# Beryl2000/SE-UNet-AirSeg

Measured on AMD Instinct MI355X. Metric: voxels/sec SE-UNet fwd+bwd, 128^3 patch, higher is better.
Workload: dtype bf16

## Files before the change

### include/seunet_hip.h

```cpp
#ifndef SEUNET_HIP_H
#define SEUNET_HIP_H
#include <stddef.h>

#ifdef __cplusplus
extern "C" {
#endif

#ifndef SEUNET_F32
#define SEUNET_F32 0
#define SEUNET_BF16 1
#define SEUNET_F16 2
#endif
#define SEUNET_CONV_MFMA 0
#define SEUNET_CONV_NAIVE 1
#define SEUNET_CONV_MARCH 2
#define SEUNET_CONV_TILED 3

typedef void* seunet_stream_t;
typedef struct seunet_dims { int n, d, h, w; } seunet_dims;

int seunet_version(void);
const char* seunet_last_error(void);
int seunet_init(int device);

// ... 50 lines not shown
                             const float* pgrad_partial, int records, float* dw_se, float* dw_se2, float* dw_side,
                             float* db_side, float* dhead_w, seunet_stream_t s);

int seunet_cat_epilogue_fwd(int dtype, const void* raw, const float* mean, const float* rstd, const void* raw2,
                            const float* mean2, const float* rstd2, int c, float slope, void* out, seunet_dims dims,
                            seunet_stream_t s);
int seunet_cat_epilogue_bwd(int dtype, const void* g_out, const void* raw, const float* mean, const float* rstd,
                            const void* raw2, const float* mean2, const float* rstd2, int c, float slope,
                            const float* m1, const float* m2, const float* m1b, const float* m2b, void* dx, void* dx2,
                            double* stat_partial, double* stat_partial2, seunet_dims dims, seunet_stream_t s);

int seunet_xbranch_moment_slots(seunet_dims dims);
int seunet_xbranch_moments(int dtype, const void* x_in, double* partial , seunet_dims dims, seunet_stream_t s);
int seunet_xbranch_stats(const double* partial, int slots, const float* w2, int c, int in_channel, int n, long long count,
                         float eps, float* mean2, float* rstd2, double* moments_out , seunet_stream_t s);
int seunet_cat_epilogue_fwd_x(int dtype, const void* raw, const float* mean, const float* rstd, const void* x_in,
                              const float* w2, int in_channel, const float* mean2, const float* rstd2, int c, float slope,
                              void* out, seunet_dims dims, seunet_stream_t s);
int seunet_cat_epilogue_bwd_x(int dtype, const void* g_out, const void* raw, const float* mean, const float* rstd,
                              const void* x_in, const float* w2, int in_channel, const float* mean2, const float* rstd2,
                              int c, float slope, const float* m1, const float* m2, const float* m1b, const float* m2b,
                              void* dx, double* stat_partial, double* stat_partial2, double* xw_partial, seunet_dims dims,
                              seunet_stream_t s);
int seunet_cat_epilogue_fwd_x_pool(int dtype, const void* raw, const float* mean, const float* rstd, const void* x_in,
                                   const float* w2, int in_channel, const float* mean2, const float* rstd2, int c, float slope,
                                   void* out, void* pooled, unsigned int* argmax, seunet_dims dims, seunet_stream_t s);
int seunet_cat_epilogue_bwd_x_pool(int dtype, const void* g_out, const void* raw, const float* mean, const float* rstd,
                                   const void* x_in, const float* w2, int in_channel, const float* mean2, const float* rstd2,
                                   int c, float slope, const float* m1, const float* m2, const float* m1b, const float* m2b,
                                   void* dx, double* stat_partial, double* stat_partial2, double* xw_partial,
// ... 235 lines not shown
```

### se-unet-airseg_amd/_lib.py

```python
from __future__ import annotations

import ctypes as C
import os
from typing import Optional, Sequence

_HERE = os.path.dirname(os.path.abspath(__file__))
LIB_PATH = os.environ.get("SEUNET_LIB") or os.path.join(_HERE, "libseunet_hip.so")

F32, BF16, F16 = 0, 1, 2
CONV_MFMA, CONV_NAIVE, CONV_MARCH, CONV_TILED = 0, 1, 2, 3
LOSS_NSUMS = 7
DTI_F64, DTI_F32 = 0, 1
CC_EVALUATION, CC_MAXIMUM_3D, CC_LARGEST_FILLED = 0, 1, 2
MORPH_DILATE, MORPH_ERODE_BORDER0, MORPH_ERODE_BORDER1, MORPH_CLOSE = 0, 1, 2, 3


class Dims(C.Structure):
    _fields_ = [("n", C.c_int), ("d", C.c_int), ("h", C.c_int), ("w", C.c_int)]


class NetDesc(C.Structure):
    _fields_ = [("batch", C.c_int), ("in_channel", C.c_int), ("n_classes", C.c_int),
                ("d", C.c_int), ("h", C.c_int), ("w", C.c_int), ("width_mult", C.c_int),
                ("dtype", C.c_int), ("conv_impl", C.c_int),
# ... 58 lines not shown
    "seunet_head_bwd_tmp_floats": (_sz, [Dims]),
    "seunet_head_bwd": (_i, [_vp, _pp, _i, _vp, _vp, Dims, _vp]),
    "seunet_loss_partial_floats": (_i, []),
    "seunet_loss_sums": (_i, [_vp, _i, _vp, _vp, _vp, _ll, _vp, _vp, _i, _vp]),
    "seunet_loss_value": (_i, [_vp, _d, _d, _d, _vp, _d, _d, _d, _vp, _vp]),
    "seunet_loss_grad": (_i, [_vp, _i, _vp, _vp, _vp, _ll, _vp, _f, _f, _f, _f, _vp, _vp, _vp]),
    "seunet_loss_sample_partial_floats": (_i, [_i]),
    "seunet_loss_sums_per_sample": (_i, [_vp, _i, _vp, _vp, _vp, _i, _ll, _vp, _vp, _i, _vp]),
    "seunet_loss_sample_values": (_i, [_vp, _i, _d, _d, _d, _vp, _vp]),
    "seunet_pool_select": (_i, [_vp, _i, _vp, _vp, _vp, _i, _vp, _vp]),
    "seunet_pool_scatter": (_i, [_vp, _i, _i, _ll, _vp, _vp, _vp, _vp, _vp, _vp, _vp, _vp, _vp]),
    "seunet_pool_gather": (_i, [_ip, _i, _i, _ll, _vp, _vp, _vp, _vp, _vp, _vp, _vp, _vp, _vp]),
    "seunet_xbranch_moment_slots": (_i, [Dims]),
    "seunet_xbranch_moments": (_i, [_i, _vp, _vp, Dims, _vp]),
    "seunet_xbranch_stats": (_i, [_vp, _i, _vp, _i, _i, _i, _ll, _f, _vp, _vp, _vp, _vp]),
    "seunet_cat_epilogue_fwd_x": (_i, [_i, _vp, _vp, _vp, _vp, _vp, _i, _vp, _vp, _i, _f, _vp, Dims, _vp]),
    "seunet_cat_epilogue_bwd_x": (_i, [_i, _vp, _vp, _vp, _vp, _vp, _vp, _i, _vp, _vp, _i, _f, _vp, _vp, _vp, _vp, _vp, _vp, _vp, _vp, Dims, _vp]),
    "seunet_cat_epilogue_fwd_x_pool": (_i, [_i, _vp, _vp, _vp, _vp, _vp, _i, _vp, _vp, _i, _f, _vp, _vp, _vp, Dims, _vp]),
    "seunet_cat_epilogue_bwd_x_pool": (_i, [_i, _vp, _vp, _vp, _vp, _vp, _vp, _i, _vp, _vp, _i, _f, _vp, _vp, _vp, _vp, _vp, _vp, _vp, _vp, _vp, _vp, Dims, _vp]),
    "seunet_cat_xgrad_finalize": (_i, [_vp, _vp, _i, _vp, _vp, _i, _i, _i, _f, _vp, _vp]),
    "seunet_cc_workspace_bytes": (_sz, [_i, _i, _i]),
    "seunet_largest_component": (_i, [_vp, _i, _i, _i, _i, _vp, _vp, _vp, _sz, _vp]),
    "seunet_metric_out_bytes": (_sz, [_i]),
    "seunet_metric_sums": (_i, [_vp, _vp, _vp, _vp, _ll, _i, _vp, _sz, _vp]),
    "seunet_value_counts": (_i, [_vp, _ll, _i, _vp, _vp]),
    "seunet_shift_clamp": (_i, [_vp, _ll, _i, _i, _i, _i, _vp, _vp]),
    "seunet_get_l_workspace_bytes": (_sz, [_i, _i, _i]),
    "seunet_get_l": (_i, [_vp, _i, _i, _i, _d, _i, _vp, _vp, _sz, _vp]),
    "seunet_mask_combine": (_i, [_vp, _vp, _ll, _i, _vp, _vp]),
    "seunet_mask_box": (_i, [_vp, _i, _i, _i, _vp, _vp]),
    "seunet_crop3d": (_i, [_vp, _i, _i, _i, _i, _ip, _vp, _vp]),
# ... 126 lines not shown
```

### se-unet-airseg_amd/csrc/abi.cpp

```cpp
#include "seunet_common.h"
#include "epilogue.h"
#include "volume.h"
#include "wgrad.h"
#include "../../include/seunet_hip.h"

using namespace seunet;

static inline Dims D(seunet_dims d) { return Dims{d.n, d.d, d.h, d.w}; }
static inline hipStream_t S(seunet_stream_t s) { return reinterpret_cast<hipStream_t>(s); }

static int make_src(int nsrc, const void* const* src, const int* src_c, SrcList& l) {
  SEUNET_CHECK(nsrc >= 1 && nsrc <= 3 && src && src_c, "bad source list");
  l = SrcList{};
  l.n = nsrc;
  for (int i = 0; i < nsrc; ++i) { l.ptr[i] = src[i]; l.C[i] = src_c[i]; }
  return 0;
}

namespace seunet { extern unsigned long long* g_conv_debug; }

extern "C" {

int seunet_debug_set_buffer(void* p) { seunet::g_conv_debug = reinterpret_cast<unsigned long long*>(p); return 0; }
int seunet_debug_upsample2_form(int dtype, int c, seunet_dims dims, int backward) { return upsample2_form(dtype, c, D(dims), backward != 0); }
// ... 297 lines not shown
                       float* label_out, float* weight_out, float* skel_out, seunet_stream_t s) {
  return launch_pool_gather(slots_host, n, capacity, voxels, pool_data, pool_label, pool_weight, pool_skel, data_out, label_out,
                            weight_out, skel_out, S(s));
}

int seunet_xbranch_moment_slots(seunet_dims dims) { return xbranch_moment_slots(D(dims)); }
int seunet_xbranch_moments(int dtype, const void* x_in, double* partial, seunet_dims dims, seunet_stream_t s) {
  SEUNET_CHECK(x_in && partial, "xbranch_moments: null argument");
  return launch_xbranch_moments(dtype, x_in, partial, D(dims), S(s));
}
int seunet_xbranch_stats(const double* partial, int slots, const float* w2, int c, int in_channel, int n, long long count,
                         float eps, float* mean2, float* rstd2, double* moments_out, seunet_stream_t s) {
  SEUNET_CHECK(partial && w2 && mean2 && rstd2 && slots >= 1 && c >= 1 && n >= 1 && count >= 1, "xbranch_stats: bad argument");
  return launch_xbranch_stats(partial, slots, w2, c, in_channel, n, count, eps, mean2, rstd2, moments_out, S(s));
}
int seunet_cat_epilogue_fwd_x(int dtype, const void* raw, const float* mean, const float* rstd, const void* x_in,
                              const float* w2, int in_channel, const float* mean2, const float* rstd2, int c, float slope,
                              void* out, seunet_dims dims, seunet_stream_t s) {
  SEUNET_CHECK(raw && mean && rstd && x_in && w2 && mean2 && rstd2 && out, "cat_epilogue_fwd_x: null argument");
  const CatBlock b{{raw, mean, rstd}, {Branch2::Recomputed, x_in, mean2, rstd2, w2, in_channel}, c, slope};
  return launch_cat_fwd(dtype, b, out, PoolOut{}, D(dims), S(s));
}
int seunet_cat_epilogue_bwd_x(int dtype, const void* g_out, const void* raw, const float* mean, const float* rstd,
                              const void* x_in, const float* w2, int in_channel, const float* mean2, const float* rstd2,
                              int c, float slope, const float* m1, const float* m2, const float* m1b, const float* m2b,
                              void* dx, double* stat_partial, double* stat_partial2, double* xw_partial, seunet_dims dims,
                              seunet_stream_t s) {
  SEUNET_CHECK(g_out && raw && mean && rstd && x_in && w2 && mean2 && rstd2, "cat_epilogue_bwd_x: null argument");
  const CatBlock b{{raw, mean, rstd}, {Branch2::Recomputed, x_in, mean2, rstd2, w2, in_channel}, c, slope};
  return cat_epilogue_bwd(dtype, b, g_out, PoolGrad{}, m1, m2, m1b, m2b, dx, nullptr, stat_partial, stat_partial2, xw_partial, dims, s);
// ... 288 lines not shown
```

### se-unet-airseg_amd/csrc/cat.hip

```cpp
#include "epilogue.h"
#include "wgrad.h"
#include <type_traits>

namespace seunet {

template <bool XR>
__device__ __forceinline__ void second_branch(const float (&in8)[8], const float (&wa)[8], const float (&wb)[8], float (&x2)[8]) {
#pragma unroll
  for (int j = 0; j < 8; ++j) x2[j] = XR ? wa[j] * in8[0] + wb[j] * in8[1] : in8[j];
}

template <typename T, int LPV, bool TWO, bool XR>
__global__ void __launch_bounds__(EPI_THREADS)
cat_fwd_kernel(const T* __restrict__ raw, const float* __restrict__ mean, const float* __restrict__ rstd,
               const T* __restrict__ raw2, const float* __restrict__ mean2, const float* __restrict__ rstd2, int C, float slope,
               T* __restrict__ out, long long V, const float* __restrict__ w2x, int xic) {
  SEUNET_EPI_THREAD(LPV);
  float mu[8], rs[8], mu2[8], rs2[8], wa[8], wb[8];
#pragma unroll
  for (int j = 0; j < 8; ++j) {
    mu[j] = mean[n * C + c0 + j]; rs[j] = rstd[n * C + c0 + j];
    mu2[j] = TWO ? mean2[n * C + c0 + j] : 0.f;
    rs2[j] = TWO ? rstd2[n * C + c0 + j] : 0.f;
    wa[j] = XR ? w2x[(c0 + j) * xic] : 0.f;
// ... 255 lines not shown
__global__ void __launch_bounds__(EPI_THREADS)
input_moments_kernel(const T* __restrict__ xin, double* __restrict__ partial, long long V) {
  const int n = blockIdx.y, P = gridDim.x;
  double s[5] = {0.0, 0.0, 0.0, 0.0, 0.0};
  for (long long v = (long long)blockIdx.x * EPI_THREADS + threadIdx.x; v < V; v += (long long)P * EPI_THREADS) {
    float x[8];
    load8(xin + ((long long)n * V + v) * 8, x);
    const double a = (double)x[0], b = (double)x[1];
    s[0] += a; s[1] += b; s[2] += a * a; s[3] += a * b; s[4] += b * b;
  }
  __shared__ double red[4][5];
  block_sum(s, red);
  if (const int k = threadIdx.x; k < 5) partial[((long long)n * P + blockIdx.x) * 5 + k] = wave4_sum(red, k);
}

__global__ void __launch_bounds__(256)
xbranch_stats_kernel(const double* __restrict__ partial, int slots, const float* __restrict__ w2, int C, int ic,
                     double inv_count, float eps, float* __restrict__ mean2, float* __restrict__ rstd2,
                     double* __restrict__ moments_out) {
  const int n = blockIdx.x;
  __shared__ double red[4][5], tot[5];
  double s[5] = {0.0, 0.0, 0.0, 0.0, 0.0};
  for (int b = threadIdx.x; b < slots; b += 256)
#pragma unroll
    for (int k = 0; k < 5; ++k) s[k] += partial[((long long)n * slots + b) * 5 + k];
  block_sum(s, red);
  if (threadIdx.x < 5) tot[threadIdx.x] = wave4_sum(red, threadIdx.x) * inv_count;
  __syncthreads();
  if (moments_out != nullptr && threadIdx.x < 5) moments_out[n * 5 + threadIdx.x] = tot[threadIdx.x];
  const double m0 = tot[0], m1 = tot[1];
  const double c00 = tot[2] - m0 * m0, c01 = tot[3] - m0 * m1, c11 = tot[4] - m1 * m1;
  for (int c = threadIdx.x; c < C; c += 256) {
    const double a = (double)w2[c * ic], b = ic > 1 ? (double)w2[c * ic + 1] : 0.0;
    const double mu = a * m0 + b * m1;
    double var = a * a * c00 + 2.0 * a * b * c01 + b * b * c11;
    if (var < 0.0) var = 0.0;
    mean2[n * C + c] = (float)mu;
    rstd2[n * C + c] = (float)(1.0 / sqrt(var + (double)eps));
  }
}

__device__ __forceinline__ void
xw_finalize_body(int c, const double* __restrict__ xw_partial, const double* __restrict__ stat_partial2, int slots, int C, int N,
                 const double* __restrict__ moments, const float* __restrict__ w2, int ic, double eps, float* __restrict__ dw) {
  const int wave = threadIdx.x >> 6, lane = threadIdx.x & 63;
  __shared__ double red[4][3];
  const double wa = (double)w2[c * ic], wb = ic > 1 ? (double)w2[c * ic + 1] : 0.0;
  double g0 = 0.0, g1 = 0.0;
  for (int n = 0; n < N; ++n) {
    double s[3] = {0.0, 0.0, 0.0};
    for (int r = threadIdx.x; r < slots; r += 256) {
      const long long rec = (long long)n * slots + r;
      s[0] += xw_partial[(rec * C + c) * 2 + 0];
      s[1] += xw_partial[(rec * C + c) * 2 + 1];
// ... 171 lines not shown
int launch_xbranch_moments(int dtype, const void* x_in, double* partial, Dims d, hipStream_t s) {
  dim3 grid(xbranch_moment_slots(d), d.N);
  SEUNET_DTYPE_SWITCH(dtype, input_moments_kernel<T><<<grid, EPI_THREADS, 0, s>>>((const T*)x_in, partial, d.vox()));
  SEUNET_LAUNCH_CHECK();
  return 0;
}

int launch_xbranch_stats(const double* partial, int slots, const float* w2, int C, int in_channel, int N, long long count,
                         float eps, float* mean2, float* rstd2, double* moments_out, hipStream_t s) {
  SEUNET_CHECK(in_channel >= 1 && in_channel <= 2, "xbranch_stats: in_channel %d (1 or 2)", in_channel);
  xbranch_stats_kernel<<<N, 256, 0, s>>>(partial, slots, w2, C, in_channel, 1.0 / (double)count, eps, mean2, rstd2, moments_out);
  SEUNET_LAUNCH_CHECK();
  return 0;
}

int launch_cat_xgrad_finalize(const double* xw_partial, const double* stat_partial2, int slots, const double* moments, const float* w2,
                              int C, int in_channel, int N, float eps, float* dw, hipStream_t s) {
  SEUNET_CHECK(in_channel >= 1 && in_channel <= 2, "cat_xgrad_finalize: in_channel %d (1 or 2)", in_channel);
  xw_finalize_kernel<<<C, 256, 0, s>>>(xw_partial, stat_partial2, slots, C, N, moments, w2, in_channel, (double)eps, dw);
  SEUNET_LAUNCH_CHECK();
  return 0;
}

int launch_cat_bwd_finalize(const double* stat_partial, const double* stat_partial2, int slots, int C, int N, long long count,
                            float* m1, float* m2, float* m1b, float* m2b, const CatXwFinalize& xw, hipStream_t s,
                            const WgReduceJob* rider) {
  SEUNET_CHECK(stat_partial && m1 && m2 && (!stat_partial2 || (m1b && m2b)), "cat_bwd_finalize: missing argument");
  SEUNET_CHECK(!xw.dw || (stat_partial2 && xw.xw_partial && xw.moments && xw.w2 && xw.in_channel >= 1 && xw.in_channel <= 2),
               "cat_bwd_finalize: the x-branch weight gradient needs the second branch's sums and in_channel 1 or 2");
  const WgReduceJob job = rider ? *rider : WgReduceJob{};
// ... 19 lines not shown
```

### se-unet-airseg_amd/csrc/epilogue.h

```cpp
#pragma once
#include "seunet_common.h"

namespace seunet {

struct WgReduceJob;
int epi_partials(Dims d);
int launch_channel_stats(int dtype, const void* t, int C, double* partial, Dims d, hipStream_t s);
int launch_stats_finalize(const double* partial, int slots, int C, int N, long long count,
                          float eps, int mode, float* out_a, float* out_b, hipStream_t s);
struct NormIn { const void* raw; const float* mean; const float* rstd; };
struct SseParams {
  const float* w_se;
  const float* w_se2;
  const float* w_side;
  const float* b_side;
  float slope;
};
struct GateBlock { NormIn a; int C; SseParams p; };
struct SseHead {
  float* side_out;
  float* level_map;
  int level_accumulate;
  const float* head_w;
  const float* drop;
// ... 37 lines not shown
  const float *m1, *m2, *m1b, *m2b;
  void* dx;
  void* dx2;
  float* gx_out;
  int gx_acc;
};
int launch_cat_fwd(int dtype, const CatBlock& b, void* out, const PoolOut& pool, Dims d, hipStream_t s);
int launch_cat_bwd_sums(int dtype, const CatBlock& b, const void* g_out, const PoolGrad& pool, const CatSums& out, Dims d,
                        hipStream_t s);
int launch_cat_bwd_apply(int dtype, const CatBlock& b, const void* g_out, const PoolGrad& pool, const CatApply& io, Dims d,
                         hipStream_t s);
int xbranch_moment_slots(Dims d);
int launch_xbranch_moments(int dtype, const void* x_in, double* partial, Dims d, hipStream_t s);
int launch_xbranch_stats(const double* partial, int slots, const float* w2, int C, int in_channel, int N, long long count,
                         float eps, float* mean2, float* rstd2, double* moments_out, hipStream_t s);
int launch_cat_xgrad_finalize(const double* xw_partial, const double* stat_partial2, int slots, const double* moments, const float* w2,
                              int C, int in_channel, int N, float eps, float* dw, hipStream_t s);
struct CatXwFinalize { const double* xw_partial; const double* moments; const float* w2; int in_channel; float eps; float* dw; };
int launch_cat_bwd_finalize(const double* stat_partial, const double* stat_partial2, int slots, int C, int N, long long count,
                            float* m1, float* m2, float* m1b, float* m2b, const CatXwFinalize& xw, hipStream_t s,
                            const WgReduceJob* rider = nullptr);
int launch_xbranch_values(int dtype, const void* x_in, const float* w2, int C, int in_channel, float* out_ncdhw, Dims d, hipStream_t s);

#ifdef __HIPCC__
static constexpr int EPI_THREADS = 256;

template <typename T> __device__ __forceinline__ float round_to(float v) {
  if constexpr (sizeof(T) == 4) return v;
  else return unpack_lo<T>(pack2<T>(v, 0.f));
}
// ... 87 lines not shown
```

### se-unet-airseg_amd/csrc/net.cpp

```cpp
#include "seunet_common.h"
#include "epilogue.h"
#include "wgrad.h"
#include "../../include/seunet_hip.h"

#include <algorithm>
#include <cstdio>
#include <cstring>
#include <string>
#include <vector>

namespace seunet {

ConvKernel wgrad_kernel(int dtype, int taps, int dil, const SrcList& x, int cin_logical, int cout, Dims d, long long src_dist) {
  if (taps == 1) {
    const int combos = cdiv(cin_logical, 32) * cdiv(cout, 32);
    const long long nv = (long long)d.N * d.vox();
    const bool pays = combos >= 16 || (combos >= 8 && nv >= 500000);
    return pays && wgrad_1x1_supported(dtype, x, cin_logical, cout) ? ConvKernel::Wgrad1x1 : ConvKernel::Tiled;
  }
  const bool fine = d.W >= 32 && (long long)d.D * d.H * d.W >= 48LL * 48 * 48;
  const bool pays = fine || dil == 2 || cin_logical >= 256;
  return pays && wgrad_march_supported(dtype, taps, dil, x, cin_logical, cout, d, src_dist) ? ConvKernel::March : ConvKernel::Tiled;
}

namespace {

bool g_wgrad_defer = true;

enum TId {
  T_NONE,
  T_X0, T_X1, T_X2,
  T_E0, T_E1A, T_E1_1, T_E1, T_E2IN, T_E2, T_E3A, T_E3_1, T_E3, T_E4IN, T_E4, T_E5A, T_E5_1, T_E5,
  T_E6IN, T_E6, T_E7A, T_E7_1, T_E7, T_E8, T_D0A, T_D0_1, T_D0, T_D1U, T_D1A, T_D1_1, T_D1, T_D2U, T_D2A, T_D2_1,
  T_COUNT
};
enum OpKind { OP_GATED, OP_CAT, OP_POOL, OP_UP };
struct OpDesc {
  OpKind kind; const char* name;
  int src[3]; int dst;
  int cout;
  int dil; int gates;
  const char* xname; int xsrc;
// ... 116 lines not shown

struct Take { const char* what; const char* of; size_t off, bytes; };
constexpr const char* kDigit[] = {"0", "1", "2", "3"};

struct Plan {
  seunet_net_desc d;
  size_t esz;
  Dims dims[4];
  int C[T_COUNT];
  size_t feat[T_COUNT], grad[T_COUNT];
  OpRes op[kNumOps];
  size_t lvl[2][4], glvl[2][4];
  size_t stats, stats2, pgrad, m1, m2, m1b, m2b, wgrad_ws, head_tmp, gx, xwp = 0, xmom = 0;
  size_t gside = 0, cls_part = 0, cls_bias = 0;
  bool fuse_x = false;
  size_t wgrad_ws_bytes;
  size_t total;
  size_t ig_gx[3] = {0, 0, 0}, ig_total = 0;

  size_t cur = 0;
  std::vector<Take> log;
  size_t take(size_t bytes, const char* what, const char* of = "") {
    log.push_back({what, of, cur, bytes});
    cur = align_up(cur + bytes, 256);
    return log.back().off;
  }

  const Dims& dims_of(int t) const { return dims[kG.level[t]]; }
  long long src_dist(int i) const {
    return kG.nsrc[i] == 2 ? (long long)feat[kOps[i].src[1]] - (long long)feat[kOps[i].src[0]] : 0;
  }
// ... 98 lines not shown
      slots_max = std::max(slots_max, std::max(std::max(conv_stats_tiles(dm, 27, 1), conv_stats_tiles(dm, 27, 2)), epi_partials(dm)));
      cmax = std::max(cmax, r.cout);
      if (d.n_classes > 1 && o.kind == OP_GATED) r.side = take((size_t)d.batch * dm.vox() * 2 * 4, "side", o.name);
    }
    for (int h = 0; h < 2; ++h)
      for (int l = 0; l < 4; ++l) {
        lvl[h][l] = take((size_t)d.n_classes * d.batch * dims[l].vox() * 4, h ? "lvl.dec" : "lvl.enc", kDigit[l]);
        glvl[h][l] = take((size_t)d.n_classes * d.batch * dims[l].vox() * 4, h ? "glvl.dec" : "glvl.enc", kDigit[l]);
      }
    if (d.n_classes > 1) {
      gside = take((size_t)d.batch * dims[0].vox() * 2 * 4, "gside");
      cls_part = take((size_t)d.batch * 256 * 2 * d.n_classes * 8, "cls_part");
      cls_bias = take((size_t)d.batch * d.n_classes * 4, "cls_bias");
    }
    const size_t stat_bytes = (size_t)d.batch * slots_max * cmax * 2 * 8;
    stats = take(stat_bytes, "stats");
    stats2 = take(stat_bytes, "stats2");
    pgrad = take((size_t)d.batch * slots_max * (4 * cmax + 4) * 4, "pgrad");
    m1 = take((size_t)d.batch * cmax * 4, "m1");
    m2 = take((size_t)d.batch * cmax * 4, "m2");
    m1b = take((size_t)d.batch * cmax * 4, "m1b");
    m2b = take((size_t)d.batch * cmax * 4, "m2b");
    wgrad_ws_bytes = wg_max;
    wgrad_ws = take(wg_max, "wgrad_ws");
    head_tmp = take(head_bwd_tmp_floats(dims[0]) * 4, "head_tmp");
    gx = take(gx_max, "gx");
    xwp = take(xw_max, "xwp");
    xmom = take(xmom_max, "xmom");
    total = cur;
    cur = 0;
// ... 176 lines not shown
                               c.r.raw, c.r.cout, c.r.mean, c.r.rstd, c.dm)) return e;
    const SseHead hd = sse_head(c.i, !lvl_written[h][c.lv]);
    lvl_written[h][c.lv] = true;
    mark("epi_fwd:", c.o.name);
    if (int e = launch_sse_fwd(p.d.dtype, gate_block(c), at(p.feat[c.o.dst]), hd, c.dm, s)) return e;
    return hd.side_out ? side_to_level(c, hd.level_accumulate) : 0;
  }

  int cat_forward(const Op& c) {
    const OpRes& r = c.r;
    const CatBlock blk = cat_block(c);
    if (int e = conv_and_stats(c.o.name, r.fwd, 1, 1, srcs(c.i), r.cin, par(c.i, P_CONV1_W), nullptr, r.wp_f, r.raw, r.cout, r.mean,
                               r.rstd, c.dm)) return e;
    PoolOut pool_out{};
    if (blk.b.kind == Branch2::Recomputed) {
      mark("stats");
      if (int e = launch_xbranch_moments(p.d.dtype, blk.b.src, dat(p.xmom), c.dm, s)) return e;
      if (int e = launch_xbranch_stats(dat(p.xmom), xbranch_moment_slots(c.dm), blk.b.w2, r.cout, p.d.in_channel, c.dm.N, c.dm.vox(),
                                       p.d.eps, fat(r.mean2), fat(r.rstd2), dat(r.xtot), s)) return e;
      SEUNET_CHECK(r.fused >= 0, "net: internal: %s has no max-pool to write", c.o.name);
      pool_out = PoolOut{at(p.feat[kOps[r.fused].dst]), reinterpret_cast<unsigned*>(at(p.op[r.fused].pool_idx))};
    } else if (blk.b.kind == Branch2::Stored) {
      if (int e = conv_and_stats(c.o.xname, r.x_fwd, 1, 1, xbranch_src(c.o), p.d.in_channel, par(kG.prm[c.i].xw), nullptr, r.wp_x, r.raw2,
                                 r.cout, r.mean2, r.rstd2, c.dm)) return e;
    }
    mark("cat_fwd:", c.o.name);
    return launch_cat_fwd(p.d.dtype, blk, at(p.feat[c.o.dst]), pool_out, c.dm, s);
  }

  int pool_forward(const Op& c) {
    if (c.r.fused >= 0) return 0;
    const int t = c.o.src[0];
    mark("pool_fwd:", c.o.name);
    return launch_maxpool_fwd(p.d.dtype, at(p.feat[t]), p.C[t], at(p.feat[c.o.dst]), p.dims_of(t), s);
  }

  int up_forward(const Op& c) {
    const int t = c.o.src[0];
    mark("up_fwd:", c.o.name);
    return launch_upsample2_fwd(p.d.dtype, at(p.feat[t]), p.C[t], at(p.feat[c.o.dst]), p.dims_of(t), s);
  }

  int heads_forward(float* pred0, float* pred1) {
    float* const pred[2] = {pred0, pred1};
    const Dims d1{1, p.dims[0].D, p.dims[0].H, p.dims[0].W};
    mark("head_fwd");
// ... 1 lines not shown
      if (pred[h] == nullptr) continue;
      const int nl = 4 - h;
      if (p.d.n_classes > 1) {
        if (int e = per_sample_class(p.lvl[h], 0, nl, [&](float* const* lm, size_t nc) {
              return launch_head_fwd(lm, nl, par(kG.head_b[h]) + nc % p.d.n_classes, pred[h] + nc * d1.vox(), d1, s);
            })) return e;
      } else {
        const float* lm[4] = {fat(p.lvl[h][0]), fat(p.lvl[h][1]), fat(p.lvl[h][2]), fat(p.lvl[h][3])};
        if (int e = launch_head_fwd(lm, nl, par(kG.head_b[h]), pred[h], p.dims[0], s)) return e;
      }
    }
    mark("outside");
    return 0;
  }

  int forward(const float* x, const float* drop1, const float* drop2, float* pred0, float* pred1) {
    skip_enc_head = pred0 == nullptr;
    drops[0] = drop1; drops[1] = drop2;
    if (int e = pack_all_weights(false)) return e;
    mark("pack_input");
    if (int e = launch_pack_input(p.d.dtype, x, p.d.in_channel, at(p.feat[T_X0]), p.dims[0], s)) return e;
    for (int i = 0; i < kNumOps; ++i) {
      const Op c = op(i);
      const OpKind k = c.o.kind;
      if (int e = k == OP_GATED ? gated_forward(c) : k == OP_CAT ? cat_forward(c) : k == OP_POOL ? pool_forward(c) : up_forward(c))
        return e;
    }
    return heads_forward(pred0, pred1);
  }

  const float* g_pred[2] = {nullptr, nullptr};
  float* const* grads = nullptr;
  bool written[T_COUNT] = {};
  std::vector<float*> zero_ptrs;
  std::vector<int> zero_counts;
  hipEvent_t decoder_done = nullptr;
// ... 216 lines not shown
  if (int e = p.init(*desc)) return e;
  if (index < 0 || index >= (int)p.log.size()) return 1;
  const Take& t = p.log[index];
  snprintf(name, (size_t)cap, "%s%s%s", t.what, t.of[0] ? ":" : "", t.of);
  *offset = t.off;
  *bytes = t.bytes;
  return 0;
}

int seunet_debug_net_wgrad_defer(int on) {
  const int was = g_wgrad_defer ? 1 : 0;
  g_wgrad_defer = on != 0;
  return was;
}

int seunet_net_forward(const seunet_net_desc* desc, const float* const* params, const float* x, const float* drop1,
                       const float* drop2, float* pred0, float* pred1, void* workspace, size_t workspace_bytes,
                       seunet_stream_t s) {
  SEUNET_CHECK(x && pred1, "net_forward: null tensor");
  Exec ex;
  if (int e = ex.setup(desc, params, workspace, workspace_bytes, (hipStream_t)s)) return e;
  return ex.forward(x, drop1, drop2, pred0, pred1);
}

struct NetGraph {
  hipGraph_t graph = nullptr;
  hipGraphExec_t exec = nullptr;
};

int seunet_net_forward_capture(const seunet_net_desc* desc, const float* const* params, const float* x, const float* drop1,
// ... 151 lines not shown
```

### se-unet-airseg_amd/ops.py

```python
from __future__ import annotations

import ctypes as C
from typing import List, Optional, Sequence, Tuple

import torch

from . import _lib
from ._lib import Dims


def _tdtype(code: int):
    return {_lib.BF16: torch.bfloat16, _lib.F16: torch.float16}.get(code, torch.float32)


def _code(t: torch.Tensor) -> int:
    return {torch.bfloat16: _lib.BF16, torch.float16: _lib.F16}.get(t.dtype, _lib.F32)


def _dims_cl(t: torch.Tensor) -> Dims:
    n, d, h, w, _ = t.shape
    return Dims(n, d, h, w)


def _s():
# ... 270 lines not shown
    n, d, h, w, _ = x_in.shape
    dims = _dims_cl(x_in)
    c = w2.shape[0]
    w2f = w2.contiguous().float().reshape(c, in_channel)
    mslots = lib.seunet_xbranch_moment_slots(dims)
    mom = torch.zeros((n, mslots, 5), dtype=torch.float64, device=x_in.device)
    _lib.check(lib.seunet_xbranch_moments(_code(x_in), x_in.data_ptr(), mom.data_ptr(), dims, _s()), "xbranch_moments")
    mean2 = torch.empty((n, c), dtype=torch.float32, device=x_in.device)
    rstd2 = torch.empty_like(mean2)
    tot = torch.empty((n, 5), dtype=torch.float64, device=x_in.device)
    _lib.check(lib.seunet_xbranch_stats(mom.data_ptr(), mslots, w2f.data_ptr(), c, in_channel, n, d * h * w, eps, mean2.data_ptr(),
                                        rstd2.data_ptr(), tot.data_ptr(), _s()), "xbranch_stats")
    return mean2, rstd2, tot


def cat_epilogue_fwd_x(raw, mean, rstd, x_in, w2, in_channel, mean2, rstd2, slope=0.01):
    c = raw.shape[4]
    w2f = w2.contiguous().float().reshape(c, in_channel)
    out = torch.empty_like(raw)
    _lib.check(_lib.load().seunet_cat_epilogue_fwd_x(_code(raw), raw.data_ptr(), mean.data_ptr(), rstd.data_ptr(), x_in.data_ptr(),
                                                     w2f.data_ptr(), in_channel, mean2.data_ptr(), rstd2.data_ptr(), c, slope,
                                                     out.data_ptr(), _dims_cl(raw), _s()), "cat_epilogue_fwd_x")
    return out


def cat_epilogue_fwd_x_pool(raw, mean, rstd, x_in, w2, in_channel, mean2, rstd2, slope=0.01):
    n, d, h, w, c = raw.shape
    w2f = w2.contiguous().float().reshape(c, in_channel)
    out = torch.empty_like(raw)
    pooled = torch.empty((n, d // 2, h // 2, w // 2, c), dtype=raw.dtype, device=raw.device)
# ... 200 lines not shown
```

Baseline: 586.0 million.

## Fuse input packing, two max-pool levels and x-branch moments into one pyramid kernel

Adds a kernel that reads the fp32 NCDHW input once. It writes the packed level-0 tensor plus the 2x and 4x max-pooled levels, and accumulates per-level x-branch moment records in the same pass. A single batched stats kernel then finalizes the mean and rstd for all three levels, replacing the separate pack, pool and per-level moment/stat launches. This cuts repeated passes over the input pyramid and several small launches, at the cost of a register-heavy kernel that needs extents divisible by 4 and reuses the stats buffer as scratch.

```diff
diff --git a/include/seunet_hip.h b/include/seunet_hip.h
--- a/include/seunet_hip.h
+++ b/include/seunet_hip.h
@@ -88,6 +88,12 @@
 int seunet_xbranch_moments(int dtype, const void* x_in, double* partial , seunet_dims dims, seunet_stream_t s);
 int seunet_xbranch_stats(const double* partial, int slots, const float* w2, int c, int in_channel, int n, long long count,
                          float eps, float* mean2, float* rstd2, double* moments_out , seunet_stream_t s);
+int seunet_input_pyramid_slots(seunet_dims dims);
+int seunet_input_pyramid(int dtype, const float* x, int in_channel, void* x0, void* x1, void* x2, double* partial, seunet_dims dims,
+                         seunet_stream_t s);
+int seunet_xbranch_stats_levels(const double* partial, int slots, const float* const* w2, const int* c, int in_channel,
+                                seunet_dims dims, float eps, float* const* mean2, float* const* rstd2, double* const* moments_out,
+                                seunet_stream_t s);
 int seunet_cat_epilogue_fwd_x(int dtype, const void* raw, const float* mean, const float* rstd, const void* x_in,
                               const float* w2, int in_channel, const float* mean2, const float* rstd2, int c, float slope,
                               void* out, seunet_dims dims, seunet_stream_t s);
diff --git a/se-unet-airseg_amd/_lib.py b/se-unet-airseg_amd/_lib.py
--- a/se-unet-airseg_amd/_lib.py
+++ b/se-unet-airseg_amd/_lib.py
@@ -96,7 +96,10 @@
     "seunet_xbranch_moment_slots": (_i, [Dims]),
     "seunet_xbranch_moments": (_i, [_i, _vp, _vp, Dims, _vp]),
     "seunet_xbranch_stats": (_i, [_vp, _i, _vp, _i, _i, _i, _ll, _f, _vp, _vp, _vp, _vp]),
-    "seunet_cat_epilogue_fwd_x": (_i, [_i, _vp, _vp, _vp, _vp, _vp, _i, _vp, _vp, _i, _f, _vp, Dims, _vp]),
+    "seunet_input_pyramid_slots": (_i, [Dims]),
+    "seunet_input_pyramid": (_i, [_i, _vp, _i, _vp, _vp, _vp, _vp, Dims, _vp]),
+    "seunet_xbranch_stats_levels": (_i, [_vp, _i, _pp, _ip, _i, Dims, _f, _pp, _pp, _pp, _vp]),
+    "seunet_cat_epilogue_fwd_x":(_i, [_i, _vp, _vp, _vp, _vp, _vp, _i, _vp, _vp, _i, _f, _vp, Dims, _vp]),
     "seunet_cat_epilogue_bwd_x": (_i, [_i, _vp, _vp, _vp, _vp, _vp, _vp, _i, _vp, _vp, _i, _f, _vp, _vp, _vp, _vp, _vp, _vp, _vp, _vp, Dims, _vp]),
     "seunet_cat_epilogue_fwd_x_pool": (_i, [_i, _vp, _vp, _vp, _vp, _vp, _i, _vp, _vp, _i, _f, _vp, _vp, _vp, Dims, _vp]),
     "seunet_cat_epilogue_bwd_x_pool": (_i, [_i, _vp, _vp, _vp, _vp, _vp, _vp, _i, _vp, _vp, _i, _f, _vp, _vp, _vp, _vp, _vp, _vp, _vp, _vp, _vp, _vp, Dims, _vp]),
diff --git a/se-unet-airseg_amd/csrc/abi.cpp b/se-unet-airseg_amd/csrc/abi.cpp
--- a/se-unet-airseg_amd/csrc/abi.cpp
+++ b/se-unet-airseg_amd/csrc/abi.cpp
@@ -335,6 +335,34 @@
   SEUNET_CHECK(partial && w2 && mean2 && rstd2 && slots >= 1 && c >= 1 && n >= 1 && count >= 1, "xbranch_stats: bad argument");
   return launch_xbranch_stats(partial, slots, w2, c, in_channel, n, count, eps, mean2, rstd2, moments_out, S(s));
 }
+int seunet_input_pyramid_slots(seunet_dims dims) {
+  if (dims.d < 4 || dims.h < 4 || dims.w < 4 || dims.d % 4 || dims.h % 4 || dims.w % 4) {
+    (void)fail("input_pyramid_slots: extents (%d, %d, %d) must be multiples of 4", dims.d, dims.h, dims.w);
+    return 0;
+  }
+  return input_pyramid_slots(D(dims));
+}
+int seunet_input_pyramid(int dtype, const float* x, int in_channel, void* x0, void* x1, void* x2, double* partial, seunet_dims dims,
+                         seunet_stream_t s) {
+  SEUNET_CHECK(x && x0 && x1 && x2 && partial && dtype_ok(dtype), "input_pyramid: bad argument");
+  return launch_input_pyramid(dtype, x, in_channel, x0, x1, x2, partial, D(dims), S(s));
+}
+int seunet_xbranch_stats_levels(const double* partial, int slots, const float* const* w2, const int* c, int in_channel,
+                                seunet_dims dims, float eps, float* const* mean2, float* const* rstd2, double* const* moments_out,
+                                seunet_stream_t s) {
+  SEUNET_CHECK(partial && w2 && c && mean2 && rstd2 && slots >= 1 && dims.n >= 1, "xbranch_stats_levels: bad argument");
+  XStatsLevels lv{};
+  for (int l = 0; l < 3; ++l) {
+    lv.partial[l] = partial + (size_t)l * dims.n * slots * 5;
+    lv.w2[l] = w2[l];
+    lv.C[l] = c[l];
+    lv.inv_count[l] = 1.0 / (double)(D(dims).vox() >> (3 * l));
+    lv.mean2[l] = mean2[l];
+    lv.rstd2[l] = rstd2[l];
+    lv.moments_out[l] = moments_out ? moments_out[l] : nullptr;
+  }
+  return launch_xbranch_stats_levels(lv, 3, slots, in_channel, dims.n, eps, S(s));
+}
 int seunet_cat_epilogue_fwd_x(int dtype, const void* raw, const float* mean, const float* rstd, const void* x_in,
                               const float* w2, int in_channel, const float* mean2, const float* rstd2, int c, float slope,
                               void* out, seunet_dims dims, seunet_stream_t s) {
diff --git a/se-unet-airseg_amd/csrc/cat.hip b/se-unet-airseg_amd/csrc/cat.hip
--- a/se-unet-airseg_amd/csrc/cat.hip
+++ b/se-unet-airseg_amd/csrc/cat.hip
@@ -293,11 +293,10 @@
   if (const int k = threadIdx.x; k < 5) partial[((long long)n * P + blockIdx.x) * 5 + k] = wave4_sum(red, k);
 }
 
-__global__ void __launch_bounds__(256)
-xbranch_stats_kernel(const double* __restrict__ partial, int slots, const float* __restrict__ w2, int C, int ic,
-                     double inv_count, float eps, float* __restrict__ mean2, float* __restrict__ rstd2,
-                     double* __restrict__ moments_out) {
-  const int n = blockIdx.x;
+__device__ __forceinline__ void
+xbranch_stats_body(int n, const double* __restrict__ partial, int slots, const float* __restrict__ w2, int C, int ic,
+                   double inv_count, float eps, float* __restrict__ mean2, float* __restrict__ rstd2,
+                   double* __restrict__ moments_out) {
   __shared__ double red[4][5], tot[5];
   double s[5] = {0.0, 0.0, 0.0, 0.0, 0.0};
   for (int b = threadIdx.x; b < slots; b += 256)
@@ -317,6 +316,17 @@
     mean2[n * C + c] = (float)mu;
     rstd2[n * C + c] = (float)(1.0 / sqrt(var + (double)eps));
   }
+}
+__global__ void __launch_bounds__(256)
+xbranch_stats_kernel(const double* __restrict__ partial, int slots, const float* __restrict__ w2, int C, int ic,
+                     double inv_count, float eps, float* __restrict__ mean2, float* __restrict__ rstd2,
+                     double* __restrict__ moments_out) {
+  xbranch_stats_body(blockIdx.x, partial, slots, w2, C, ic, inv_count, eps, mean2, rstd2, moments_out);
+}
+__global__ void __launch_bounds__(256) xbranch_stats_levels_kernel(XStatsLevels lv, int slots, int ic, float eps) {
+  const int l = blockIdx.y;
+  xbranch_stats_body(blockIdx.x, lv.partial[l], slots, lv.w2[l], lv.C[l], ic, lv.inv_count[l], eps, lv.mean2[l], lv.rstd2[l],
+                     lv.moments_out[l]);
 }
 
 __device__ __forceinline__ void
@@ -518,6 +528,16 @@
   return 0;
 }
 
+int launch_xbranch_stats_levels(const XStatsLevels& lv, int nlevels, int slots, int in_channel, int N, float eps, hipStream_t s) {
+  SEUNET_CHECK(in_channel >= 1 && in_channel <= 2, "xbranch_stats_levels: in_channel %d (1 or 2)", in_channel);
+  SEUNET_CHECK(nlevels >= 1 && nlevels <= 3 && slots >= 1 && N >= 1, "xbranch_stats_levels: bad argument");
+  for (int l = 0; l < nlevels; ++l)
+    SEUNET_CHECK(lv.partial[l] && lv.w2[l] && lv.mean2[l] && lv.rstd2[l] && lv.C[l] >= 1, "xbranch_stats_levels: level %d lacks an argument", l);
+  xbranch_stats_levels_kernel<<<dim3(N, nlevels), 256, 0, s>>>(lv, slots, in_channel, eps);
+  SEUNET_LAUNCH_CHECK();
+  return 0;
+}
+
 int launch_cat_xgrad_finalize(const double* xw_partial, const double* stat_partial2, int slots, const double* moments, const float* w2,
                               int C, int in_channel, int N, float eps, float* dw, hipStream_t s) {
   SEUNET_CHECK(in_channel >= 1 && in_channel <= 2, "cat_xgrad_finalize: in_channel %d (1 or 2)", in_channel);
diff --git a/se-unet-airseg_amd/csrc/epilogue.h b/se-unet-airseg_amd/csrc/epilogue.h
--- a/se-unet-airseg_amd/csrc/epilogue.h
+++ b/se-unet-airseg_amd/csrc/epilogue.h
@@ -75,6 +75,14 @@
 int launch_xbranch_moments(int dtype, const void* x_in, double* partial, Dims d, hipStream_t s);
 int launch_xbranch_stats(const double* partial, int slots, const float* w2, int C, int in_channel, int N, long long count,
                          float eps, float* mean2, float* rstd2, double* moments_out, hipStream_t s);
+int input_pyramid_slots(Dims d);
+int launch_input_pyramid(int dtype, const float* x_ncdhw, int in_channel, void* X0, void* X1, void* X2, double* partial, Dims d,
+                         hipStream_t s);
+struct XStatsLevels {
+  const double* partial[3]; const float* w2[3]; int C[3]; double inv_count[3];
+  float* mean2[3]; float* rstd2[3]; double* moments_out[3];
+};
+int launch_xbranch_stats_levels(const XStatsLevels& lv, int nlevels, int slots, int in_channel, int N, float eps, hipStream_t s);
 int launch_cat_xgrad_finalize(const double* xw_partial, const double* stat_partial2, int slots, const double* moments, const float* w2,
                               int C, int in_channel, int N, float eps, float* dw, hipStream_t s);
 struct CatXwFinalize { const double* xw_partial; const double* moments; const float* w2; int in_channel; float eps; float* dw; };
diff --git a/se-unet-airseg_amd/csrc/input_pyramid.hip b/se-unet-airseg_amd/csrc/input_pyramid.hip
--- /dev/null
+++ b/se-unet-airseg_amd/csrc/input_pyramid.hip
@@ -0,0 +1,146 @@
+#include "seunet_common.h"
+#include "epilogue.h"
+
+namespace seunet {
+
+static constexpr int PYR_THREADS = 256;
+
+__device__ __forceinline__ float f4_at(const float4& v, int i) { return i == 0 ? v.x : i == 1 ? v.y : i == 2 ? v.z : v.w; }
+
+template <typename T, int IC>
+__global__ void __launch_bounds__(PYR_THREADS)
+input_pyramid_kernel(const float* __restrict__ x, T* __restrict__ X0, T* __restrict__ X1, T* __restrict__ X2,
+                     double* __restrict__ partial, int D, int H, int W) {
+  __shared__ float stage[4][4][IC][PYR_THREADS];
+  __shared__ double red[4][15];
+  const int n = blockIdx.y, N = gridDim.y, slots = gridDim.x;
+  const int wave = threadIdx.x >> 6, lane = threadIdx.x & 63;
+  const int Wc = W >> 2, Hc = H >> 2, cells = (D >> 2) * Hc * Wc;
+  const int H1 = H >> 1, W1 = W >> 1;
+  const long long V = (long long)D * H * W;
+  const int cell = blockIdx.x * PYR_THREADS + threadIdx.x;
+  const bool live = cell < cells;
+  const int xc = cell % Wc, yc = (cell / Wc) % Hc, zc = cell / (Wc * Hc);
+
+  float4 v[IC][4][4];
+  if (live) {
+    const float* src = x + (long long)n * IC * V + ((long long)(4 * zc) * H + 4 * yc) * W + 4 * xc;
+#pragma unroll
+    for (int c = 0; c < IC; ++c)
+#pragma unroll
+      for (int z = 0; z < 4; ++z)
+#pragma unroll
+        for (int y = 0; y < 4; ++y) v[c][z][y] = *reinterpret_cast<const float4*>(src + c * V + ((long long)z * H + y) * W);
+  }
+
+  long long sv[4];
+  bool slive[4];
+#pragma unroll
+  for (int j = 0; j < 4; ++j) {
+    const int cj = blockIdx.x * PYR_THREADS + wave * 64 + 16 * j + (lane >> 2);
+    slive[j] = cj < cells;
+    const int xj = cj % Wc, yj = (cj / Wc) % Hc, zj = cj / (Wc * Hc);
+    sv[j] = (long long)n * V + ((long long)(4 * zj) * H + 4 * yj) * W + 4 * xj + (lane & 3);
+  }
+
+  double s[15];
+#pragma unroll
+  for (int k = 0; k < 15; ++k) s[k] = 0.0;
+  float m1[IC][2][2], m2[IC];
+#pragma unroll
+  for (int c = 0; c < IC; ++c) m2[c] = -INFINITY;
+
+#pragma unroll
+  for (int z = 0; z < 4; ++z) {
+    if (live) {
+      if ((z & 1) == 0) {
+#pragma unroll
+        for (int c = 0; c < IC; ++c)
+#pragma unroll
+          for (int k = 0; k < 4; ++k) m1[c][k >> 1][k & 1] = -INFINITY;
+      }
+#pragma unroll
+      for (int y = 0; y < 4; ++y) {
+        float r[IC][4];
+#pragma unroll
+        for (int i = 0; i < 4; ++i) {
+#pragma unroll
+          for (int c = 0; c < IC; ++c) {
+            r[c][i] = round_to<T>(f4_at(v[c][z][y], i));
+            float& m = m1[c][y >> 1][i >> 1];
+            m = r[c][i] > m ? r[c][i] : m;
+          }
+          const double a = (double)r[0][i], b = IC > 1 ? (double)r[IC - 1][i] : 0.0;
+          s[0] += a; s[1] += b; s[2] += a * a; s[3] += a * b; s[4] += b * b;
+        }
+#pragma unroll
+        for (int c = 0; c < IC; ++c)
+          *reinterpret_cast<float4*>(&stage[wave][y][c][4 * lane]) = make_float4(r[c][0], r[c][1], r[c][2], r[c][3]);
+      }
+    }
+    __builtin_amdgcn_wave_barrier();
+#pragma unroll
+    for (int y = 0; y < 4; ++y)
+#pragma unroll
+      for (int j = 0; j < 4; ++j) {
+        if (!slive[j]) continue;
+        float o[8];
+#pragma unroll
+        for (int c = 0; c < 8; ++c) o[c] = c < IC ? stage[wave][y][c < IC ? c : 0][64 * j + lane] : 0.f;
+        store8(X0 + (sv[j] + ((long long)z * H + y) * W) * 8, o);
+      }
+    __builtin_amdgcn_wave_barrier();
+    if (live && (z & 1)) {
+      const int z1 = 2 * zc + (z >> 1);
+#pragma unroll
+      for (int yy = 0; yy < 2; ++yy)
+#pragma unroll
+        for (int xx = 0; xx < 2; ++xx) {
+          float o[8];
+#pragma unroll
+          for (int c = 0; c < 8; ++c) o[c] = c < IC ? m1[c < IC ? c : 0][yy][xx] : 0.f;
+#pragma unroll
+          for (int c = 0; c < IC; ++c) m2[c] = o[c] > m2[c] ? o[c] : m2[c];
+          const double a = (double)o[0], b = IC > 1 ? (double)o[1] : 0.0;
+          s[5] += a; s[6] += b; s[7] += a * a; s[8] += a * b; s[9] += b * b;
+          const long long v1 = (long long)n * (V >> 3) + ((long long)z1 * H1 + 2 * yc + yy) * W1 + 2 * xc + xx;
+          store8(X1 + v1 * 8, o);
+        }
+    }
+  }
+  if (live) {
+    float o[8];
+#pragma unroll
+    for (int c = 0; c < 8; ++c) o[c] = c < IC ? m2[c < IC ? c : 0] : 0.f;
+    const double a = (double)o[0], b = IC > 1 ? (double)o[1] : 0.0;
+    s[10] = a; s[11] = b; s[12] = a * a; s[13] = a * b; s[14] = b * b;
+    store8(X2 + ((long long)n * (V >> 6) + cell) * 8, o);
+  }
+  block_sum(s, red);
+  if (const int k = threadIdx.x; k < 15) {
+    const int l = k / 5;
+    partial[(((long long)l * N + n) * slots + blockIdx.x) * 5 + (k - 5 * l)] = wave4_sum(red, k);
+  }
+}
+
+int input_pyramid_slots(Dims d) { return cdiv((d.D / 4) * (d.H / 4) * (d.W / 4), PYR_THREADS); }
+
+static inline bool aligned16(const void* p) { return (reinterpret_cast<uintptr_t>(p) & 15) == 0; }
+
+int launch_input_pyramid(int dtype, const float* x, int in_channel, void* X0, void* X1, void* X2, double* partial, Dims d,
+                         hipStream_t s) {
+  SEUNET_CHECK(in_channel >= 1 && in_channel <= 2, "input_pyramid: in_channel %d (1 or 2)", in_channel);
+  SEUNET_CHECK(d.N >= 1 && d.N <= 65535 && d.D >= 4 && d.H >= 4 && d.W >= 4 && d.D % 4 == 0 && d.H % 4 == 0 && d.W % 4 == 0,
+               "input_pyramid: extents (%d, %d, %d, %d) must be multiples of 4", d.N, d.D, d.H, d.W);
+  SEUNET_CHECK(d.vox() / 64 < (1ll << 30), "input_pyramid: %lld voxels per sample is too many", d.vox());
+  SEUNET_CHECK(aligned16(x) && aligned16(X0) && aligned16(X1) && aligned16(X2), "input_pyramid: every tensor must be 16-byte aligned");
+  const dim3 grid(input_pyramid_slots(d), d.N);
+  SEUNET_DTYPE_SWITCH(dtype, {
+    if (in_channel == 1) input_pyramid_kernel<T, 1><<<grid, PYR_THREADS, 0, s>>>(x, (T*)X0, (T*)X1, (T*)X2, partial, d.D, d.H, d.W);
+    else input_pyramid_kernel<T, 2><<<grid, PYR_THREADS, 0, s>>>(x, (T*)X0, (T*)X1, (T*)X2, partial, d.D, d.H, d.W);
+  });
+  SEUNET_LAUNCH_CHECK();
+  return 0;
+}
+
+}
diff --git a/se-unet-airseg_amd/csrc/net.cpp b/se-unet-airseg_amd/csrc/net.cpp
--- a/se-unet-airseg_amd/csrc/net.cpp
+++ b/se-unet-airseg_amd/csrc/net.cpp
@@ -26,6 +26,7 @@
 namespace {
 
 bool g_wgrad_defer = true;
+bool g_input_pyramid = true;
 
 enum TId {
   T_NONE,
@@ -172,7 +173,7 @@
   size_t stats, stats2, pgrad, m1, m2, m1b, m2b, wgrad_ws, head_tmp, gx, xwp = 0, xmom = 0;
   size_t gside = 0, cls_part = 0, cls_bias = 0;
   bool fuse_x = false;
-  size_t wgrad_ws_bytes;
+  size_t wgrad_ws_bytes, stats_bytes;
   size_t total;
   size_t ig_gx[3] = {0, 0, 0}, ig_total = 0;
 
@@ -301,6 +302,7 @@
       cls_bias = take((size_t)d.batch * d.n_classes * 4, "cls_bias");
     }
     const size_t stat_bytes = (size_t)d.batch * slots_max * cmax * 2 * 8;
+    stats_bytes = stat_bytes;
     stats = take(stat_bytes, "stats");
     stats2 = take(stat_bytes, "stats2");
     pgrad = take((size_t)d.batch * slots_max * (4 * cmax + 4) * 4, "pgrad");
@@ -507,10 +509,12 @@
                                r.rstd, c.dm)) return e;
     PoolOut pool_out{};
     if (blk.b.kind == Branch2::Recomputed) {
-      mark("stats");
-      if (int e = launch_xbranch_moments(p.d.dtype, blk.b.src, dat(p.xmom), c.dm, s)) return e;
-      if (int e = launch_xbranch_stats(dat(p.xmom), xbranch_moment_slots(c.dm), blk.b.w2, r.cout, p.d.in_channel, c.dm.N, c.dm.vox(),
-                                       p.d.eps, fat(r.mean2), fat(r.rstd2), dat(r.xtot), s)) return e;
+      if (!pyramid) {
+        mark("stats");
+        if (int e = launch_xbranch_moments(p.d.dtype, blk.b.src, dat(p.xmom), c.dm, s)) return e;
+        if (int e = launch_xbranch_stats(dat(p.xmom), xbranch_moment_slots(c.dm), blk.b.w2, r.cout, p.d.in_channel, c.dm.N, c.dm.vox(),
+                                         p.d.eps, fat(r.mean2), fat(r.rstd2), dat(r.xtot), s)) return e;
+      }
       SEUNET_CHECK(r.fused >= 0, "net: internal: %s has no max-pool to write", c.o.name);
       pool_out = PoolOut{at(p.feat[kOps[r.fused].dst]), reinterpret_cast<unsigned*>(at(p.op[r.fused].pool_idx))};
     } else if (blk.b.kind == Branch2::Stored) {
@@ -523,6 +527,7 @@
 
   int pool_forward(const Op& c) {
     if (c.r.fused >= 0) return 0;
+    if (pyramid && is_input(c.o.src[0])) return 0;
     const int t = c.o.src[0];
     mark("pool_fwd:", c.o.name);
     return launch_maxpool_fwd(p.d.dtype, at(p.feat[t]), p.C[t], at(p.feat[c.o.dst]), p.dims_of(t), s);
@@ -554,12 +559,47 @@
     return 0;
   }
 
+  bool pyramid = false;
+  int input_pyramid(const float* x) {
+    const Dims& d0 = p.dims[0];
+    const int slots = input_pyramid_slots(d0);
+    const size_t level_doubles = (size_t)d0.N * slots * 5;
+    SEUNET_CHECK(3 * level_doubles * 8 <= p.stats_bytes, "net: the input pyramid's %zu bytes of records exceed the statistics buffer (%zu)",
+                 3 * level_doubles * 8, p.stats_bytes);
+    if (int e = launch_input_pyramid(p.d.dtype, x, p.d.in_channel, at(p.feat[T_X0]), at(p.feat[T_X1]), at(p.feat[T_X2]), dat(p.stats),
+                                     d0, s)) return e;
+    XStatsLevels lv{};
+    int found = 0;
+    for (int i = 0; i < kNumOps; ++i) {
+      const Op c = op(i);
+      if (c.o.kind != OP_CAT || !c.o.xname) continue;
+      const int l = kG.level[c.o.xsrc];
+      SEUNET_CHECK(l >= 0 && l < 3 && is_input(c.o.xsrc) && !lv.partial[l], "net: internal: x-branch %s is not on a level of the pyramid", c.o.xname);
+      lv.partial[l] = dat(p.stats) + l * level_doubles;
+      lv.w2[l] = par(kG.prm[i].xw);
+      lv.C[l] = c.r.cout;
+      lv.inv_count[l] = 1.0 / (double)c.dm.vox();
+      lv.mean2[l] = fat(c.r.mean2);
+      lv.rstd2[l] = fat(c.r.rstd2);
+      lv.moments_out[l] = dat(c.r.xtot);
+      ++found;
+    }
+    SEUNET_CHECK(found == 3, "net: internal: %d x-branches for the pyramid's three levels", found);
+    mark("stats");
+    return launch_xbranch_stats_levels(lv, 3, slots, p.d.in_channel, d0.N, p.d.eps, s);
+  }
+
   int forward(const float* x, const float* drop1, const float* drop2, float* pred0, float* pred1) {
     skip_enc_head = pred0 == nullptr;
     drops[0] = drop1; drops[1] = drop2;
     if (int e = pack_all_weights(false)) return e;
+    pyramid = g_input_pyramid && p.fuse_x;
     mark("pack_input");
-    if (int e = launch_pack_input(p.d.dtype, x, p.d.in_channel, at(p.feat[T_X0]), p.dims[0], s)) return e;
+    if (pyramid) {
+      if (int e = input_pyramid(x)) return e;
+    } else {
+      if (int e = launch_pack_input(p.d.dtype, x, p.d.in_channel, at(p.feat[T_X0]), p.dims[0], s)) return e;
+    }
     for (int i = 0; i < kNumOps; ++i) {
       const Op c = op(i);
       const OpKind k = c.o.kind;
@@ -806,6 +846,12 @@
   return was;
 }
 
+int seunet_debug_net_input_pyramid(int on) {
+  const int was = g_input_pyramid ? 1 : 0;
+  g_input_pyramid = on != 0;
+  return was;
+}
+
 int seunet_net_forward(const seunet_net_desc* desc, const float* const* params, const float* x, const float* drop1,
                        const float* drop2, float* pred0, float* pred1, void* workspace, size_t workspace_bytes,
                        seunet_stream_t s) {
diff --git a/se-unet-airseg_amd/ops.py b/se-unet-airseg_amd/ops.py
--- a/se-unet-airseg_amd/ops.py
+++ b/se-unet-airseg_amd/ops.py
@@ -308,6 +308,37 @@
     return mean2, rstd2, tot
 
 
+def input_pyramid(x: torch.Tensor, dtype="bf16"):
+    lib = _lib.load()
+    code = dtype if isinstance(dtype, int) else _lib.dtype_code(dtype)
+    x = x.contiguous().float()
+    n, c, d, h, w = x.shape
+    dims = Dims(n, d, h, w)
+    slots = lib.seunet_input_pyramid_slots(dims)
+    if slots < 1:
+        raise RuntimeError(f"libseunet_hip input_pyramid_slots: {_lib.last_error()}")
+    xs = [torch.empty((n, d >> l, h >> l, w >> l, 8), dtype=_tdtype(code), device=x.device) for l in range(3)]
+    rec = torch.empty((3, n, slots, 5), dtype=torch.float64, device=x.device)
+    _lib.check(lib.seunet_input_pyramid(code, x.data_ptr(), c, xs[0].data_ptr(), xs[1].data_ptr(), xs[2].data_ptr(), rec.data_ptr(),
+                                        dims, _s()), "input_pyramid")
+    return xs[0], xs[1], xs[2], rec
+
+
+def xbranch_stats_levels(records, w2s, in_channel, dims0, eps=1e-5):
+    lib = _lib.load()
+    _, n, slots, _ = records.shape
+    dev = records.device
+    cs = [int(w.shape[0]) for w in w2s]
+    w2f = [w.contiguous().float().reshape(c, in_channel) for w, c in zip(w2s, cs)]
+    mean2 = [torch.empty((n, c), dtype=torch.float32, device=dev) for c in cs]
+    rstd2 = [torch.empty((n, c), dtype=torch.float32, device=dev) for c in cs]
+    tot = [torch.empty((n, 5), dtype=torch.float64, device=dev) for _ in cs]
+    _lib.check(lib.seunet_xbranch_stats_levels(records.data_ptr(), slots, _lib.ptr_array(w2f), _lib.int_array(cs), in_channel,
+                                               Dims(*dims0), eps, _lib.ptr_array(mean2), _lib.ptr_array(rstd2), _lib.ptr_array(tot),
+                                               _s()), "xbranch_stats_levels")
+    return mean2, rstd2, tot
+
+
 def cat_epilogue_fwd_x(raw, mean, rstd, x_in, w2, in_channel, mean2, rstd2, slope=0.01):
     c = raw.shape[4]
     w2f = w2.contiguous().float().reshape(c, in_channel)
```

Result: no change. 590.7 million (median of 6 runs) (+0.8%).
